# ghostop14/gr-clenabled

Measured on AMD Instinct MI355X. Metric: MSamples/sec (complex-float) through clFFT 4096 fwd + window + shift, higher is better.
Workload: dtype f32; 1 GPU; BASELINE configs[1]: forward clFFT 4096-pt complex, blackman window + fftshift, 16384 frames/step/GPU device-resident (1 GiB in+out); fft_size=4096, parallelism=replica-per-gpu x1

## Files before the change

gr-clenabled_amd/csrc/fft.hip:

```cpp
#include <cmath>
#include <cstdlib>
#include <vector>

#include "common.h"
#include "fft_core.hpp"
#include "fft_mr.h"

using namespace fftc;
#ifndef MI355_FFT_WPE
#define MI355_FFT_WPE 3
#endif

namespace {

typedef float f2v __attribute__((ext_vector_type(2)));

template <int N, bool REAL, class G>
__device__ __forceinline__ void load_group(c32 (&v)[16], const void *__restrict__ in, int grp, int tid, int nframes, int in_xor)
{
    using P = Plan<N>;
    constexpr int TH = G::TH, PTS = G::PTS, F = G::F, R0 = P::radix(0), B0 = N / R0;
    const int frames_left = nframes - grp * F;
    if constexpr (N <= 64) {
        (void)in_xor;
// ... 496 lines not shown
template <int N>
int launch_s(mi355_ctx *ctx, int sign, const void *in, void *out, const float *window, const void *tw, int nframes, int shift,
             int real_in, hipStream_t st)
{
    const int grid = N == 32768   ? mi355_balanced_grid(ctx, nframes, 1, 1)
                     : N == 16384 ? mi355_balanced_grid(ctx, nframes, 16, 16)
                                  : mi355_balanced_grid(ctx, nframes, 4, 4);
    if constexpr (N == 32768) {
        if (!getenv("MI355_FFT_32768_IN_REGISTERS")) {
#define LAUNCH_32K(SG, RL) hipLaunchKernelGGL((k_fft_32k<SG, RL>), dim3(grid), dim3(512), 0, st, in, (c32 *)out, window, (const c32 *)tw, nframes, shift)
            if (sign < 0) { if (real_in) LAUNCH_32K(-1, true); else LAUNCH_32K(-1, false); }
            else          { if (real_in) LAUNCH_32K(1, true);  else LAUNCH_32K(1, false); }
#undef LAUNCH_32K
            MI355_HIP(hipGetLastError());
            return MI355_OK;
        }
    }
    if constexpr (N == 32768) MI355_SWITCH_NOTE(ctx, "MI355_FFT_32768_IN_REGISTERS", "k_fft_s<32768> instead of k_fft_32k");
#define LAUNCH_S(SG, RL) hipLaunchKernelGGL((k_fft_s<N, SG, RL>), dim3(grid), dim3(256), 0, st, in, (c32 *)out, window, (const c32 *)tw, nframes, shift)
    if (sign < 0) { if (real_in) LAUNCH_S(-1, true); else LAUNCH_S(-1, false); }
    else          { if (real_in) LAUNCH_S(1, true);  else LAUNCH_S(1, false); }
#undef LAUNCH_S
    MI355_HIP(hipGetLastError());
    return MI355_OK;
}

template <int SIGN, bool REAL>
__global__ __launch_bounds__(256, 2) void k_fft_sub(const void *__restrict__ in, c32 *__restrict__ ws, const float *__restrict__ window,
                                                    const c32 *__restrict__ tw4096, int S, int nquad , int in_xor)
{
    constexpr int NS = 4096, BL = 256, Q = 4;
    using G = Geo<NS>;
    __shared__ c32 lds[NS];
    const int tid0 = threadIdx.x;
    const int per = S / Q, nframes = nquad / per;
    const int xcd = blockIdx.x & 7, per_xcd = gridDim.x >> 3;
    for (int q = blockIdx.x >> 3;; q += per_xcd) {
        const int frame = (q / per) * 8 + xcd, s = Q * (q % per);
        if (q / per >= (nframes + 7) / 8) break;
        if (frame >= nframes) continue;
        int tid = tid0;
        asm volatile("" : "+v"(tid));
        const size_t fb = (size_t)frame * NS * S;
        c32 v[Q][16];
#pragma unroll
        for (int r = 0; r < 16; r++) {
            const int n = tid + ((r ^ in_xor) * BL);
            const size_t e = (size_t)n * S + s;
            const f4v w = *((const f4v *)window + (size_t)(s >> 2) * NS + n);
            if constexpr (REAL) {
                const f4v x = *(const f4v *)((const float *)in + fb + e);
                v[0][r] = mk(x.x * w.x, 0.f);
                v[1][r] = mk(x.y * w.y, 0.f);
                v[2][r] = mk(x.z * w.z, 0.f);
                v[3][r] = mk(x.w * w.w, 0.f);
            } else {
                const f4v x0 = *(const f4v *)((const c32 *)in + fb + e);
                const f4v x1 = *((const f4v *)((const c32 *)in + fb + e) + 1);
                v[0][r] = mk(x0.x * w.x, x0.y * w.x);
                v[1][r] = mk(x0.z * w.y, x0.w * w.y);
                v[2][r] = mk(x1.x * w.z, x1.y * w.z);
                v[3][r] = mk(x1.z * w.w, x1.w * w.w);
            }
        }
        TwRegs<NS> tw;
        load_twiddles<NS, false, G>(tw, tid, tw4096);
#define MI355_SUBQ(K)                                                                                                   \
        {                                                                                                              \
            transform_regs<NS, SIGN, false, G>(v[K], tw, lds, tid);                                                    \
            f2v *__restrict__ o = (f2v *)ws + ((size_t)frame * S + s + K) * NS + tid;                                  \
            _Pragma("unroll") for (int t = 0; t < 16; t++) {                                                           \
                f2v z;                                                                                                 \
                z.x = v[K][t].x;                                                                                       \
                z.y = v[K][t].y;                                                                                       \
                o[orev<16>(t) * BL] = z;                            \
            }                                                                                                          \
            __syncthreads();                                                                                           \
        }
        MI355_SUBQ(0) MI355_SUBQ(1) MI355_SUBQ(2) MI355_SUBQ(3)
#undef MI355_SUBQ
    }
}

template <int S, int SIGN>
__global__ __launch_bounds__(256) void k_fft_combine(const c32 *__restrict__ ws, c32 *__restrict__ out, const c32 *__restrict__ twN,
                                                     long long total , int m_xor)
{
    constexpr int NS = 4096, N = NS * S;
    for (long long e = (long long)blockIdx.x * 256 + threadIdx.x; e < total; e += (long long)gridDim.x * 256) {
        const long long frame = e / NS;
        const int k = (int)(e - frame * NS);
        const c32 *src = ws + (size_t)frame * N + k;
        c32 a[S];
#pragma unroll
        for (int s = 0; s < S; s++) a[s] = src[(size_t)s * NS];
        c32 wsl[tw_slots<S>()];
#pragma unroll
        for (int i = 0; i < tw_slots<S>(); i++) wsl[i] = twN[(tw_power<S>(i) * k) & (N - 1)];
        apply_twiddles<S>(a, wsl);
        bfly<S, SIGN>(a);
        f2v *dst = (f2v *)out + (size_t)frame * N + k;
#pragma unroll
        for (int t = 0; t < S; t++) {
            f2v z;
            z.x = a[t].x;
            z.y = a[t].y;
            __builtin_nontemporal_store(z, dst + (size_t)((orev<S>(t) ^ m_xor) * NS));
        }
    }
}

template <int S, int SIGN>
__global__ __launch_bounds__(256) void k_fft_combine2(const c32 *__restrict__ src, c32 *__restrict__ dst, const c32 *__restrict__ twN,
                                                      long long total , int nsub, long long frame_elems, long long src_sub,
                                                      long long src_set, long long dst_set, int tw_mul, int nmask, int m_xor)
{
    const int set = blockIdx.y;
    for (long long e = (long long)blockIdx.x * 256 + threadIdx.x; e < total; e += (long long)gridDim.x * 256) {
        const long long frame = e / nsub;
        const int k = (int)(e - frame * nsub);
        const c32 *in = src + (size_t)frame * frame_elems + (size_t)set * src_set + k;
        c32 a[S];
#pragma unroll
        for (int s = 0; s < S; s++) a[s] = in[(size_t)s * src_sub];
        c32 wsl[tw_slots<S>()];
#pragma unroll
        for (int i = 0; i < tw_slots<S>(); i++) wsl[i] = twN[(int)(((long long)tw_power<S>(i) * k * tw_mul) & nmask)];
        apply_twiddles<S>(a, wsl);
        bfly<S, SIGN>(a);
        f2v *out = (f2v *)dst + (size_t)frame * frame_elems + (size_t)set * dst_set + k;
#pragma unroll
        for (int t = 0; t < S; t++) {
            f2v z;
            z.x = a[t].x;
            z.y = a[t].y;
            out[(size_t)((orev<S>(t) ^ m_xor)) * nsub] = z;
        }
    }
}

template <int NR> struct GeoTile {
    static constexpr int TH = NR, PTS = 16 * NR, F = 16, WPE = 1;
};

template <int NR, int SIGN, bool PASS_B, bool REAL, bool WR>
__global__ __launch_bounds__(NR, 4) void k_fft_tile(const void *__restrict__ in, c32 *__restrict__ out, const float *__restrict__ window,
                                                 const c32 *__restrict__ twN, const c32 *__restrict__ twR,
                                                 int ld , int nmask ,
                                                 long long nitems , int row_xor)
{
    using G = GeoTile<NR>;
    constexpr bool REV = !PASS_B;
    using PL = Plan<NR, REV>;
    constexpr int TH = NR, CS = NR + 1;
    extern __shared__ __attribute__((aligned(16))) c32 tile_lds[];
    const int tid0 = threadIdx.x;
    TwRegs<NR> tw;
    load_twiddles<NR, REV, G>(tw, tid0, twR);
    const int tiles = ld / 16;
    const size_t frame_elems = (size_t)NR * ld;
    constexpr bool WREG = !PASS_B && WR;
    float wreg[16];
    int c0_window = -1;
    for (long long item = blockIdx.x; item < nitems; item += gridDim.x) {
        int tid = tid0;
        asm volatile("" : "+v"(tid));
        const long long frame = item / tiles;
        const int c0 = (int)(item - frame * tiles) * 16;
        if constexpr (WREG) {
            if (c0 != c0_window) {
#pragma unroll
                for (int i = 0; i < 16; i++) {
                    const int e = tid + TH * i, col = e & 15, row = e >> 4;
                    wreg[i] = window[(size_t)(row ^ row_xor) * ld + c0 + col];
                }
                c0_window = c0;
            }
        }
#pragma unroll
        for (int i = 0; i < 16; i++) {
            const int e = tid + TH * i, col = e & 15, row = e >> 4;
            const size_t idx = (size_t)(PASS_B ? row : (row ^ row_xor)) * ld + c0 + col;
            c32 x;
            if constexpr (REAL) x = mk(((const float *)in)[(size_t)frame * frame_elems + idx], 0.f);
            else {
                const f2v t = __builtin_nontemporal_load((const f2v *)in + (size_t)frame * frame_elems + idx);
                x = mk(t.x, t.y);
            }
            if constexpr (!PASS_B) {
                const float w = WREG ? wreg[i] : window[idx];
                x = mk(x.x * w, x.y * w);
            }
            tile_lds[col * CS + row] = x;
        }
        __syncthreads();
        c32 v[16];
        constexpr int R0 = PL::radix(0), B0 = NR / R0;
#pragma unroll
        for (int q = 0; q < 16 / R0; q++) {
            const int g = tid + TH * q, fr = g / B0, j = g % B0;
#pragma unroll
            for (int r = 0; r < R0; r++) v[q * R0 + r] = tile_lds[fr * CS + j + r * B0];
        }
        __syncthreads();
        transform_regs<NR, SIGN, REV, G>(v, tw, tile_lds, tid);
        constexpr int NP = PL::NP, RL = PL::radix(NP - 1), BL = NR / RL;
        if constexpr (!PASS_B) {
            static_assert(RL == 16, "reversed plan: the last pass is radix 16");
            const int fr = tid / BL, j = tid % BL, n2 = c0 + fr;
            const c32 base = twN[(int)(((long long)n2 * j) & nmask)], g1 = twN[(int)(((long long)n2 * BL) & nmask)];
            const c32 g2 = cmul(g1, g1), g4 = cmul(g2, g2), g8 = cmul(g4, g4);
            c32 gp[16];
            gp[0] = base;
            gp[1] = cmul(base, g1);
            gp[2] = cmul(base, g2);
            gp[3] = cmul(gp[2], g1);
            gp[4] = cmul(base, g4);
            gp[5] = cmul(gp[4], g1);
            gp[6] = cmul(gp[4], g2);
            gp[7] = cmul(gp[6], g1);
#pragma unroll
            for (int m = 0; m < 8; m++) gp[8 + m] = cmul(gp[m], g8);
            f2v *__restrict__ o = (f2v *)out + (size_t)frame * frame_elems + (size_t)n2 * NR + j;
#pragma unroll
            for (int t = 0; t < 16; t++) {
                const c32 z = cmul(v[t], gp[orev<16>(t)]);
                f2v zz;
                zz.x = z.x;
                zz.y = z.y;
                o[orev<16>(t) * BL] = zz;
            }
            __syncthreads();
        } else {
            __syncthreads();
#pragma unroll
            for (int q = 0; q < 16 / RL; q++) {
                const int g = tid + TH * q, fr = g / BL, j = g % BL;
#pragma unroll
                for (int t = 0; t < RL; t++) tile_lds[fr * CS + j + orev<RL>(t) * BL] = v[q * RL + t];
            }
            __syncthreads();
#pragma unroll
            for (int i = 0; i < 16; i++) {
                const int e = tid + TH * i, col = e & 15, row = e >> 4;
                const c32 z = tile_lds[col * CS + row];
                f2v zz;
                zz.x = z.x;
                zz.y = z.y;
                __builtin_nontemporal_store(zz, (f2v *)out + (size_t)frame * frame_elems + (size_t)(row ^ row_xor) * ld + c0 + col);
            }
            __syncthreads();
        }
    }
}

template <int NR> struct GeoTileH {
    static constexpr int TH = NR / 2, PTS = 8 * NR, F = 8, WPE = 1;
};

template <int NR, int SIGN, bool PASS_B, bool REAL>
__global__ __launch_bounds__(NR / 2) void k_fft_tile_h(const void *__restrict__ in, c32 *__restrict__ out, const float *__restrict__ window,
                                                       const c32 *__restrict__ twN, const c32 *__restrict__ twR, int ld, int nmask,
                                                       long long nitems, int row_xor)
{
    using G = GeoTileH<NR>;
    constexpr bool REV = !PASS_B;
    using PL = Plan<NR, REV>;
    constexpr int TH = NR / 2, CS = NR + 1;
    extern __shared__ __attribute__((aligned(16))) c32 tile_lds[];
    const int tid0 = threadIdx.x;
    TwRegs<NR> tw;
    load_twiddles<NR, REV, G>(tw, tid0, twR);
    const int tiles = ld / 16;
    const size_t frame_elems = (size_t)NR * ld;
    auto fetch = [&](long long item, c32 (&pf)[32], int tid) {
        const long long frame = item / tiles;
        const int c0 = (int)(item - frame * tiles) * 16;
#pragma unroll
        for (int i = 0; i < 32; i++) {
            const int e = tid + TH * i, col = e & 15, row = e >> 4;
            const size_t idx = (size_t)(PASS_B ? row : (row ^ row_xor)) * ld + c0 + col;
            if constexpr (REAL) pf[i] = mk(((const float *)in)[(size_t)frame * frame_elems + idx], 0.f);
            else {
                const f2v t = __builtin_nontemporal_load((const f2v *)in + (size_t)frame * frame_elems + idx);
                pf[i] = mk(t.x, t.y);
            }
        }
    };
    c32 pf[32];
    if ((long long)blockIdx.x < nitems) fetch(blockIdx.x, pf, tid0);
    for (long long item = blockIdx.x; item < nitems; item += gridDim.x) {
        int tid = tid0;
        asm volatile("" : "+v"(tid));
        const long long frame = item / tiles;
        const int c0 = (int)(item - frame * tiles) * 16;
#pragma unroll
        for (int i = 0; i < 32; i++) {
            const int e = tid + TH * i, col = e & 15, row = e >> 4;
            c32 x = pf[i];
            if constexpr (!PASS_B) {
                const float w = window[(size_t)(row ^ row_xor) * ld + c0 + col];
                x = mk(x.x * w, x.y * w);
            }
            tile_lds[col * CS + row] = x;
        }
        __syncthreads();
        c32 va[16], vb[16];
        constexpr int R0 = PL::radix(0), B0 = NR / R0;
#pragma unroll
        for (int q = 0; q < 16 / R0; q++) {
            const int g = tid + TH * q, fr = g / B0, j = g % B0;
#pragma unroll
            for (int r = 0; r < R0; r++) {
                va[q * R0 + r] = tile_lds[fr * CS + j + r * B0];
                vb[q * R0 + r] = tile_lds[(fr + 8) * CS + j + r * B0];
            }
        }
        __syncthreads();
        if (item + gridDim.x < nitems) fetch(item + gridDim.x, pf, tid);
        transform_regs2<NR, SIGN, REV, G>(va, vb, tw, tile_lds, tile_lds + 8 * NR, tid);
        constexpr int NP = PL::NP, RL = PL::radix(NP - 1), BL = NR / RL;
        if constexpr (!PASS_B) {
            static_assert(RL == 16, "reversed plan: the last pass is radix 16");
            const int fr = tid / BL, j = tid % BL;
#pragma unroll
            for (int h = 0; h < 2; h++) {
                const int n2 = c0 + fr + 8 * h;
                const c32 base = twN[(int)(((long long)n2 * j) & nmask)], g1 = twN[(int)(((long long)n2 * BL) & nmask)];
                const c32 g2 = cmul(g1, g1), g4 = cmul(g2, g2), g8 = cmul(g4, g4);
                c32 gp[16];
                gp[0] = base;
                gp[1] = cmul(base, g1);
                gp[2] = cmul(base, g2);
                gp[3] = cmul(gp[2], g1);
                gp[4] = cmul(base, g4);
                gp[5] = cmul(gp[4], g1);
                gp[6] = cmul(gp[4], g2);
                gp[7] = cmul(gp[6], g1);
#pragma unroll
                for (int m = 0; m < 8; m++) gp[8 + m] = cmul(gp[m], g8);
                f2v *__restrict__ o = (f2v *)out + (size_t)frame * frame_elems + (size_t)n2 * NR + j;
#pragma unroll
                for (int t = 0; t < 16; t++) {
                    const c32 z = cmul(h ? vb[t] : va[t], gp[orev<16>(t)]);
                    f2v zz;
                    zz.x = z.x;
                    zz.y = z.y;
                    o[orev<16>(t) * BL] = zz;
                }
            }
            __syncthreads();
        } else {
            __syncthreads();
#pragma unroll
            for (int q = 0; q < 16 / RL; q++) {
                const int g = tid + TH * q, fr = g / BL, j = g % BL;
#pragma unroll
                for (int t = 0; t < RL; t++) {
                    tile_lds[fr * CS + j + orev<RL>(t) * BL] = va[q * RL + t];
                    tile_lds[(fr + 8) * CS + j + orev<RL>(t) * BL] = vb[q * RL + t];
                }
            }
            __syncthreads();
#pragma unroll
            for (int i = 0; i < 32; i++) {
                const int e = tid + TH * i, col = e & 15, row = e >> 4;
                const c32 z = tile_lds[col * CS + row];
                f2v zz;
                zz.x = z.x;
                zz.y = z.y;
                __builtin_nontemporal_store(zz, (f2v *)out + (size_t)frame * frame_elems + (size_t)(row ^ row_xor) * ld + c0 + col);
            }
            __syncthreads();
        }
    }
}

unsigned long long *stamps_buffer(int grid)
{
    static std::mutex mu;
    static unsigned long long *d = nullptr;
    static int cap = 0;
    std::lock_guard<std::mutex> g(mu);
    if (cap < grid) {
        if (d) (void)hipFree(d);
        d = nullptr;
        cap = 0;
        if (hipMalloc(&d, (size_t)grid * kTsSlots * 8) != hipSuccess) return nullptr;
        cap = grid;
    }
    return d;
}

int dump_stamps(const unsigned long long *d_ts, int n, int sign, int sched, int grid, int ngroups, hipStream_t st)
{
    MI355_HIP(hipStreamSynchronize(st));
    std::vector<unsigned long long> h((size_t)grid * kTsSlots);
    MI355_HIP(hipMemcpy(h.data(), d_ts, h.size() * 8, hipMemcpyDeviceToHost));
    unsigned long long t0 = ~0ull, t1 = 0;
    for (int b = 0; b < grid; b++) {
        t0 = std::min(t0, h[(size_t)b * kTsSlots]);
        t1 = std::max(t1, h[(size_t)b * kTsSlots + 1]);
    }
    fprintf(stderr, "[fft stamps] N %d sign %d sched %d: %d workgroups, %d groups, first start to last end %.2f us\n", n, sign, sched, grid,
            ngroups, (double)(t1 - t0) * 0.01);
    if (const char *path = getenv("MI355_FFT_TS_FILE")) {
        if (FILE *f = fopen(path, "a")) {
            fprintf(f, "# n %d sign %d sched %d grid %d ngroups %d\n", n, sign, sched, grid, ngroups);
            for (int b = 0; b < grid; b++) {
                const unsigned long long *r = &h[(size_t)b * kTsSlots];
                fprintf(f, "%d %llu %llu %llu %llu", b, r[3], r[0], r[1], r[2]);
                for (int i = 8; i < kTsSlots && r[i]; i++) fprintf(f, " %llu", r[i]);
                fprintf(f, "\n");
            }
            fclose(f);
        }
    }
    return MI355_OK;
}

template <int N, class G>
int launch_g(mi355_ctx *ctx, int sign, const void *in, void *out, const float *window, const void *tw, int nframes, int shift,
             int real_in, hipStream_t st, unsigned *claims)
{
    constexpr int F = G::F, TH = G::TH, WAVES = TH / 64;
    int ngroups = (nframes + F - 1) / F;
    int cus = ctx->num_cus > 0 ? ctx->num_cus : 256;
    int pf = getenv("MI355_FFT_PREFETCH") ? atoi(getenv("MI355_FFT_PREFETCH")) : -1;
    const bool persistent2 = N <= 4096 && WAVES == 4 && ngroups >= cus * 2 * 8;
    if (pf < 0) pf = persistent2 ? 1 : 0;
    int grid = (N <= 4096) ? mi355_balanced_grid(ctx, ngroups, 32 / WAVES, 64 / WAVES, 0.015) : mi355_balanced_grid(ctx, ngroups, 1, 1);
    if (pf == 1 && persistent2) grid = cus * 2;
    if (const char *e = getenv("MI355_FFT_WG_PER_CU")) {
        if (atoi(e) > 0) grid = ngroups < cus * atoi(e) ? ngroups : cus * atoi(e);
    }
    int sched = getenv("MI355_FFT_SCHED") ? atoi(getenv("MI355_FFT_SCHED")) : (N == 4096 ? 1 : 0);
    if (!(pf == 1 && persistent2 && claims && grid >= 8 * kClaimWords &&
          ngroups / kClaimWords >= kClaimStatic * ((grid + 8 * kClaimWords - 1) / (8 * kClaimWords)) * 8))
        sched = 0;
    if (sched != 1) claims = nullptr;
    unsigned long long *ts = nullptr;
    if (pf == 1 && getenv("MI355_FFT_TS")) {
        ts = stamps_buffer(grid);
        if (ts) MI355_HIP(hipMemsetAsync(ts, 0, (size_t)grid * kTsSlots * 8, st));
    }
#define LAUNCH_FFT_K(...) hipLaunchKernelGGL((k_fft<__VA_ARGS__>), dim3(grid), dim3(TH), 0, st, in, (c32 *)out, window, (const c32 *)tw, \
                                                nframes, ngroups, shift, claims, ts)
#define LAUNCH_FFT(SG, RL)                                                                      \
    do {                                                                                             \
        if (pf == 2) LAUNCH_FFT_K(N, SG, RL, 2, G);                                                  \
        else if (pf == 1 && sched == 1 && ts) LAUNCH_FFT_K(N, SG, RL, 1, G, true, true);             \
        else if (pf == 1 && sched == 1) LAUNCH_FFT_K(N, SG, RL, 1, G, true);                         \
        else if (pf == 1 && ts) LAUNCH_FFT_K(N, SG, RL, 1, G, false, true);                          \
        else if (pf == 1) LAUNCH_FFT_K(N, SG, RL, 1, G);                                             \
        else LAUNCH_FFT_K(N, SG, RL, 0, G);                                                          \
    } while (0)
    if (sign < 0) { if (real_in) LAUNCH_FFT(-1, true); else LAUNCH_FFT(-1, false); }
    else          { if (real_in) LAUNCH_FFT(1, true);  else LAUNCH_FFT(1, false); }
#undef LAUNCH_FFT
#undef LAUNCH_FFT_K
    MI355_HIP(hipGetLastError());
    if (ts) return dump_stamps(ts, N, sign, sched, grid, ngroups, st);
    return MI355_OK;
}

template <int N>
int launch_n(mi355_ctx *ctx, int sign, const void *in, void *out, const float *window, const void *tw, int nframes, int shift,
             int real_in, hipStream_t st, unsigned *claims)
{
    if constexpr (N >= 16 && N <= 1024) {
        static const bool wave = getenv("MI355_FFT_WAVE_GEO") ? atoi(getenv("MI355_FFT_WAVE_GEO")) != 0 : false;
        if (wave) MI355_SWITCH_NOTE(ctx, "MI355_FFT_WAVE_GEO", "k_fft in one-wave workgroups");
        if (wave) return launch_g<N, GeoW<N>>(ctx, sign, in, out, window, tw, nframes, shift, real_in, st, claims);
    }
    if constexpr (N == 32768) return launch_s<N>(ctx, sign, in, out, window, tw, nframes, shift, real_in, st);
    else if constexpr (N == 8192 || N == 16384) {
        static const bool whole = getenv("MI355_FFT_WHOLE_FRAME") ? atoi(getenv("MI355_FFT_WHOLE_FRAME")) != 0 : false;
        if (!whole) return launch_s<N>(ctx, sign, in, out, window, tw, nframes, shift, real_in, st);
        MI355_SWITCH_NOTE(ctx, "MI355_FFT_WHOLE_FRAME", "k_fft with the whole frame in LDS instead of k_fft_s");
    }
    if constexpr (N != 32768) return launch_g<N, Geo<N>>(ctx, sign, in, out, window, tw, nframes, shift, real_in, st, claims);
}

int launch_fft(mi355_ctx *ctx, int n, int sign, const void *in, void *out, const float *window, const void *tw, int nframes,
               int shift, int real_in, hipStream_t st, unsigned *claims = nullptr)
{
    switch (n) {
#define CASE_N(NN) case NN: return launch_n<NN>(ctx, sign, in, out, window, tw, nframes, shift, real_in, st, claims)
        CASE_N(2); CASE_N(4); CASE_N(8); CASE_N(16); CASE_N(32); CASE_N(64); CASE_N(128); CASE_N(256); CASE_N(512);
        CASE_N(1024); CASE_N(2048); CASE_N(4096); CASE_N(8192); CASE_N(16384); CASE_N(32768);
#undef CASE_N
    }
    mi355_set_error("fft size %d unsupported (power of two, 2..32768)", n);
    return MI355_ERR_UNSUPPORTED;
}

}

struct mi355_fft {
    mi355_ctx *ctx;
    int n, sign, dtype, nstreams, shift;
    float *d_window;
    void *d_tw;
    HostPipe pipe;
    MrPlan mr;
    MrTilePlan mrt;
    int m = 0;
    void *d_pre = nullptr, *d_post = nullptr, *d_bspec = nullptr;
    void *d_twm_f = nullptr, *d_twm_i = nullptr;
    float *d_ones = nullptr;
    mi355_fft *sub_f = nullptr, *sub_i = nullptr;
    void *d_wa = nullptr, *d_wb = nullptr;
    size_t cap_frames = 0;
    bool two_kernel = false;
    int tile_n1 = 0, tile_n2 = 0;
    std::mutex ws_lock;
    hipEvent_t ws_done = nullptr;
    bool ws_used = false;
    unsigned *d_claims = nullptr;
    hipStream_t claim_st[kClaimSets] = {};
// ... 83 lines not shown
                    if constexpr (REAL) x = mk(((const float *)in)[(fbase + fr) * N + i], 0.f);
                    else x = ((const c32 *)in)[(fbase + fr) * N + i];
                    x = cmul(x, pre[m]);
                }
                v[q * R0 + r] = x;
            }
        }
        transform_regs<M, -1, false, G>(v, twf, lds, tid);
        c32 w[16];
#pragma unroll
        for (int q = 0; q < 16 / RL; q++)
#pragma unroll
            for (int r = 0; r < RL; r++) w[q * RL + r] = cmul(v[q * RL + irev<RL>(r)], Breg[q * RL + irev<RL>(r)]);
        if constexpr (NP > 1) __syncthreads();
        if constexpr (SHARE) transform_regs<M, 1, true, G, 0, true>(w, twf, lds, tid);
        else transform_regs<M, 1, true, G>(w, twi, lds, tid);
        constexpr int RO = PI::radix(NP - 1), BO = M / RO;
#pragma unroll
        for (int q = 0; q < 16 / RO; q++) {
            const int g = tid + TH * q, fr = g / BO, j = g % BO;
#pragma unroll
            for (int t = 0; t < RO; t++) {
                const int k = j + orev<RO>(t) * BO;
                if (k < N && fr < frames_left) {
                    const int p = lo ? (k >= lo ? k - lo : k + (N - lo)) : k;
                    out[(fbase + fr) * N + p] = cmul(w[q * RO + t], post[k]);
                }
            }
        }
        if constexpr (NP > 1) __syncthreads();
    }
}

template <int M>
int launch_chirpz_m(mi355_fft *h, const void *in, void *out, int nframes, hipStream_t st)
{
    constexpr int F = Geo<M>::F, TH = Geo<M>::TH;
    const int ngroups = (nframes + F - 1) / F;
    const int grid = mi355_balanced_grid(h->ctx, ngroups, 2, 3);
    const int lo = (h->sign < 0 && h->shift) ? (h->n + 1) / 2 : 0;
    const int *src = (const int *)((const char *)h->d_post + (size_t)h->n * 8);
    constexpr int lds_bytes = Geo<M>::PTS * 8;
    if (h->dtype == MI355_DTYPE_FLOAT) {
        if (lds_bytes > 64 * 1024) MI355_HIP(hipFuncSetAttribute((const void *)k_chirpz<M, true>, hipFuncAttributeMaxDynamicSharedMemorySize, lds_bytes));
        hipLaunchKernelGGL((k_chirpz<M, true>), dim3(grid), dim3(TH), lds_bytes, st, in, (c32 *)out, (const c32 *)h->d_pre, src, (const c32 *)h->d_post,
                           (const c32 *)h->d_bspec, (const c32 *)h->d_twm_f, (const c32 *)h->d_twm_i, h->n, nframes, ngroups, lo);
    } else {
        if (lds_bytes > 64 * 1024) MI355_HIP(hipFuncSetAttribute((const void *)k_chirpz<M, false>, hipFuncAttributeMaxDynamicSharedMemorySize, lds_bytes));
        hipLaunchKernelGGL((k_chirpz<M, false>), dim3(grid), dim3(TH), lds_bytes, st, in, (c32 *)out, (const c32 *)h->d_pre, src, (const c32 *)h->d_post,
                           (const c32 *)h->d_bspec, (const c32 *)h->d_twm_f, (const c32 *)h->d_twm_i, h->n, nframes, ngroups, lo);
    }
    MI355_HIP(hipGetLastError());
    return MI355_OK;
}

int ws_acquire(mi355_fft *h, hipStream_t st, bool realloc)
{
    if (!h->ws_done) MI355_HIP(hipEventCreateWithFlags(&h->ws_done, hipEventDisableTiming));
    if (h->ws_used) {
        if (realloc) MI355_HIP(hipEventSynchronize(h->ws_done));
        else MI355_HIP(hipStreamWaitEvent(st, h->ws_done, 0));
    }
    return MI355_OK;
}
int ws_release(mi355_fft *h, hipStream_t st)
{
    MI355_HIP(hipEventRecord(h->ws_done, st));
    h->ws_used = true;
    return MI355_OK;
}

int launch_handle(mi355_fft *h, const void *in, void *out, int nvec, hipStream_t st);

int launch_bluestein(mi355_fft *h, const void *in, void *out, int nframes, hipStream_t st)
{
    const int N = h->n, M = h->m;
    static const bool fused = getenv("MI355_CHIRPZ_FUSED") ? atoi(getenv("MI355_CHIRPZ_FUSED")) != 0 : true;
    if (fused) {
        switch (M) {
        case 256: return launch_chirpz_m<256>(h, in, out, nframes, st);
        case 512: return launch_chirpz_m<512>(h, in, out, nframes, st);
        case 1024: return launch_chirpz_m<1024>(h, in, out, nframes, st);
        case 2048: return launch_chirpz_m<2048>(h, in, out, nframes, st);
        case 4096: return launch_chirpz_m<4096>(h, in, out, nframes, st);
        case 8192: return launch_chirpz_m<8192>(h, in, out, nframes, st);
        case 16384: return launch_chirpz_m<16384>(h, in, out, nframes, st);
        }
    }
    if (!fused && M >= 256 && M <= 16384) MI355_SWITCH_NOTE(h->ctx, "MI355_CHIRPZ_FUSED", "the five-launch chirp-z path instead of k_chirpz");
    size_t chunk = (128u << 20) / ((size_t)M * 8);
    if (chunk < 1) chunk = 1;
    if (chunk > (size_t)nframes) chunk = (size_t)nframes;
    std::lock_guard<std::mutex> ws_guard(h->ws_lock);
    {
        const int rc = ws_acquire(h, st, chunk > h->cap_frames);
        if (rc) return rc;
    }
    if (chunk > h->cap_frames) {
        MI355_HIP(hipStreamSynchronize(st));
        if (h->d_wa) (void)hipFree(h->d_wa);
        if (h->d_wb) (void)hipFree(h->d_wb);
        h->d_wa = h->d_wb = nullptr; h->cap_frames = 0;
        MI355_HIP(hipMalloc(&h->d_wa, chunk * (size_t)M * 8));
        MI355_HIP(hipMalloc(&h->d_wb, chunk * (size_t)M * 8));
        h->cap_frames = chunk;
    }
    const int cus = h->ctx->num_cus > 0 ? h->ctx->num_cus : 256;
    auto grid_for = [&](long long total) { long long b = (total + 255) / 256; return (unsigned)(b < (long long)cus * 16 ? b : (long long)cus * 16); };
    const size_t isz = h->dtype == MI355_DTYPE_FLOAT ? 4 : 8;
    const int len = (N + 1) / 2;
    for (size_t f0 = 0; f0 < (size_t)nframes; f0 += chunk) {
        const int nf = (int)((size_t)nframes - f0 < chunk ? (size_t)nframes - f0 : chunk);
        const long long tm = (long long)nf * M, tn = (long long)nf * N;
        hipLaunchKernelGGL(k_blu_pre, dim3(grid_for(tm)), dim3(256), 0, st, (const char *)in + f0 * N * isz, (c32 *)h->d_wa,
                           (const c32 *)h->d_pre, (const int *)((const char *)h->d_post + (size_t)N * 8), N, M, tm,
                           h->dtype == MI355_DTYPE_FLOAT ? 1 : 0);
        int rc = h->sub_f ? launch_handle(h->sub_f, h->d_wa, h->d_wb, nf, st) : launch_fft(h->ctx, M, -1, h->d_wa, h->d_wb, h->d_ones, h->d_twm_f, nf, 0, 0, st);
        if (rc) return rc;
        hipLaunchKernelGGL(k_blu_mul, dim3(grid_for(tm)), dim3(256), 0, st, (c32 *)h->d_wb, (const c32 *)h->d_bspec, M, tm);
        rc = h->sub_i ? launch_handle(h->sub_i, h->d_wb, h->d_wa, nf, st) : launch_fft(h->ctx, M, 1, h->d_wb, h->d_wa, h->d_ones, h->d_twm_i, nf, 0, 0, st);
        if (rc) return rc;
        hipLaunchKernelGGL(k_blu_post, dim3(grid_for(tn)), dim3(256), 0, st, (const c32 *)h->d_wa, (c32 *)out + f0 * N,
                           (const c32 *)h->d_post, N, M, tn, (h->sign < 0 && h->shift) ? len : 0);
        MI355_HIP(hipGetLastError());
    }
    return ws_release(h, st);
}

template <int NR, bool PASS_B>
int launch_tile(mi355_fft *h, const void *in, c32 *out, const c32 *twR, int ld, int nframes, int row_xor, bool real_in, hipStream_t st)
{
    constexpr int lds_bytes = 16 * (NR + 1) * 8;
    const int cus = h->ctx->num_cus > 0 ? h->ctx->num_cus : 256;
    const long long items = (long long)nframes * (ld / 16);
    const int per_cu = (160 * 1024) / lds_bytes;
    long long grid = (long long)cus * (per_cu < 1 ? 1 : per_cu);
    if (grid > items) grid = items;
    if (grid > ld / 16) grid -= grid % (ld / 16);
    const int nmask = h->n - 1;
    constexpr bool WRD = !PASS_B && NR == 256;
    const bool wr = !PASS_B && NR < 1024 && (getenv("MI355_FFT_TILE_WREG") ? atoi(getenv("MI355_FFT_TILE_WREG")) != 0 : WRD);
#define TILE1(SG, RL, WR)                                                                                                       \
    do {                                                                                                                        \
        MI355_HIP(hipFuncSetAttribute((const void *)k_fft_tile<NR, SG, PASS_B, RL, WR>, hipFuncAttributeMaxDynamicSharedMemorySize, lds_bytes)); \
        hipLaunchKernelGGL((k_fft_tile<NR, SG, PASS_B, RL, WR>), dim3((unsigned)grid), dim3(NR), lds_bytes, st, in, out, h->d_window, (const c32 *)h->d_tw, \
                           twR, ld, nmask, items, row_xor);                                                                     \
    } while (0)
#define TILE(SG, RL)                                                                                                            \
    do {                                                                                                                        \
        if constexpr (!PASS_B && NR < 1024) { if (wr) TILE1(SG, RL, true); else TILE1(SG, RL, false); }                         \
        else TILE1(SG, RL, false);                                                                                              \
    } while (0)
    if constexpr (NR == 1024) {
        static const bool half = getenv("MI355_FFT_TILE_HALF") ? atoi(getenv("MI355_FFT_TILE_HALF")) != 0 : true;
        if (!half) MI355_SWITCH_NOTE(h->ctx, "MI355_FFT_TILE_HALF", "k_fft_tile with one thread per sixteen values instead of k_fft_tile_h");
        if (half) {
#define TILEH(SG, RL)                                                                                                           \
    do {                                                                                                                        \
        MI355_HIP(hipFuncSetAttribute((const void *)k_fft_tile_h<NR, SG, PASS_B, RL>, hipFuncAttributeMaxDynamicSharedMemorySize, lds_bytes)); \
        hipLaunchKernelGGL((k_fft_tile_h<NR, SG, PASS_B, RL>), dim3((unsigned)grid), dim3(NR / 2), lds_bytes, st, in, out, h->d_window, (const c32 *)h->d_tw, \
                           twR, ld, nmask, items, row_xor);                                                                     \
    } while (0)
            if constexpr (PASS_B) {
                if (h->sign < 0) TILEH(-1, false); else TILEH(1, false);
            } else {
                if (h->sign < 0) { if (real_in) TILEH(-1, true); else TILEH(-1, false); }
                else             { if (real_in) TILEH(1, true);  else TILEH(1, false); }
            }
#undef TILEH
            MI355_HIP(hipGetLastError());
            return MI355_OK;
        }
    }
    if constexpr (PASS_B) {
        if (h->sign < 0) TILE(-1, false); else TILE(1, false);
    } else {
        if (h->sign < 0) { if (real_in) TILE(-1, true); else TILE(-1, false); }
        else             { if (real_in) TILE(1, true);  else TILE(1, false); }
    }
#undef TILE
#undef TILE1
    (void)wr;
    MI355_HIP(hipGetLastError());
    return MI355_OK;
}

template <bool PASS_B>
int launch_tile_nr(mi355_fft *h, int nr, const void *in, c32 *out, const c32 *twR, int ld, int nframes, int row_xor, bool real_in, hipStream_t st)
{
    switch (nr) {
    case 256: return launch_tile<256, PASS_B>(h, in, out, twR, ld, nframes, row_xor, real_in, st);
    case 512: return launch_tile<512, PASS_B>(h, in, out, twR, ld, nframes, row_xor, real_in, st);
    default: return launch_tile<1024, PASS_B>(h, in, out, twR, ld, nframes, row_xor, real_in, st);
    }
}

int launch_big(mi355_fft *h, const void *in, void *out, int nframes, hipStream_t st)
{
    const int N = h->n, S = N / 4096;
    static const size_t ws_mb = getenv("MI355_FFT_WS_MB") ? (size_t)atoi(getenv("MI355_FFT_WS_MB")) : 256;
    if (ws_mb != 256) MI355_SWITCH_NOTE(h->ctx, "MI355_FFT_WS_MB", "another workspace bound for the multi-pass sizes");
    size_t chunk = (ws_mb << 20) / ((size_t)N * 8);
    if (chunk < 1) chunk = 1;
    if (chunk > (size_t)nframes) chunk = (size_t)nframes;
    std::lock_guard<std::mutex> ws_guard(h->ws_lock);
    {
        const int rc = ws_acquire(h, st, chunk > h->cap_frames);
        if (rc) return rc;
    }
    const bool three_pass = S > 16 && !h->tile_n1;
    const bool four_pass = S > 256;
    if (chunk > h->cap_frames) {
        MI355_HIP(hipStreamSynchronize(st));
        if (h->d_wa) (void)hipFree(h->d_wa);
        if (h->d_wb) (void)hipFree(h->d_wb);
        h->d_wa = h->d_wb = nullptr; h->cap_frames = 0;
        MI355_HIP(hipMalloc(&h->d_wa, chunk * (size_t)N * 8));
        if (three_pass) MI355_HIP(hipMalloc(&h->d_wb, chunk * (size_t)N * 8));
        h->cap_frames = chunk;
    }
    const int cus = h->ctx->num_cus > 0 ? h->ctx->num_cus : 256;
    const size_t isz = h->dtype == MI355_DTYPE_FLOAT ? 4 : 8;
    const int in_xor = (h->sign > 0 && h->shift) ? 8 : 0, m_xor = (h->sign < 0 && h->shift) ? S / 2 : 0;
    const c32 *tw4096 = (const c32 *)h->d_tw + N;
    for (size_t f0 = 0; f0 < (size_t)nframes; f0 += chunk) {
        const int nf = (int)((size_t)nframes - f0 < chunk ? (size_t)nframes - f0 : chunk);
        const int nsub = nf * S / 4;
        const int grid = (mi355_balanced_grid(h->ctx, nsub, 8, 8) + 7) & ~7;
        const void *src = (const char *)in + f0 * N * isz;
        if (h->tile_n1) {
            const int n1 = h->tile_n1, n2 = h->tile_n2;
            const c32 *tw1 = (const c32 *)h->d_tw + N + 4096, *tw2 = tw1 + n1;
            int rc = launch_tile_nr<false>(h, n1, src, (c32 *)h->d_wa, tw1, n2, nf, (h->sign > 0 && h->shift) ? n1 / 2 : 0, h->dtype == MI355_DTYPE_FLOAT, st);
            if (rc) return rc;
            rc = launch_tile_nr<true>(h, n2, h->d_wa, (c32 *)out + f0 * N, tw2, n1, nf, (h->sign < 0 && h->shift) ? n2 / 2 : 0, false, st);
            if (rc) return rc;
            continue;
        }
#define SUB(SG, RL) hipLaunchKernelGGL((k_fft_sub<SG, RL>), dim3(grid), dim3(256), 0, st, src, (c32 *)h->d_wa, h->d_window, tw4096, S, nsub, in_xor)
        if (h->sign < 0) { if (h->dtype == MI355_DTYPE_FLOAT) SUB(-1, true); else SUB(-1, false); }
        else             { if (h->dtype == MI355_DTYPE_FLOAT) SUB(1, true);  else SUB(1, false); }
#undef SUB
        c32 *dst = (c32 *)out + f0 * N;
#define COMB2(SS, SG, GY, ...) hipLaunchKernelGGL((k_fft_combine2<SS, SG>), dim3((unsigned)blocks, GY), dim3(256), 0, st, __VA_ARGS__)
        if (four_pass) {
            const int S3 = S / 256, T2 = 16 * S3;
            {
                const long long total = (long long)nf * 4096;
                long long blocks = (total + 255) / 256;
                if (blocks > (long long)cus * 16 / T2 + 1) blocks = (long long)cus * 16 / T2 + 1;
                if (h->sign < 0) COMB2(16, -1, T2, (const c32 *)h->d_wa, (c32 *)h->d_wb, (const c32 *)h->d_tw, total, 4096, (long long)N, (long long)T2 * 4096, 4096LL, 65536LL, T2, N - 1, 0);
                else             COMB2(16, 1, T2, (const c32 *)h->d_wa, (c32 *)h->d_wb, (const c32 *)h->d_tw, total, 4096, (long long)N, (long long)T2 * 4096, 4096LL, 65536LL, T2, N - 1, 0);
            }
            {
                const long long total = (long long)nf * 65536;
                long long blocks = (total + 255) / 256;
                if (blocks > (long long)cus * 16 / S3 + 1) blocks = (long long)cus * 16 / S3 + 1;
                if (h->sign < 0) COMB2(16, -1, S3, (const c32 *)h->d_wb, (c32 *)h->d_wa, (const c32 *)h->d_tw, total, 65536, (long long)N, (long long)S3 * 65536, 65536LL, 1048576LL, S3, N - 1, 0);
                else             COMB2(16, 1, S3, (const c32 *)h->d_wb, (c32 *)h->d_wa, (const c32 *)h->d_tw, total, 65536, (long long)N, (long long)S3 * 65536, 65536LL, 1048576LL, S3, N - 1, 0);
            }
            {
                const long long total = (long long)nf * 1048576;
                long long blocks = (total + 255) / 256;
                if (blocks > (long long)cus * 16) blocks = (long long)cus * 16;
                const int mx = (h->sign < 0 && h->shift) ? S3 / 2 : 0;
#define COMB2G(SS) do { if (h->sign < 0) COMB2(SS, -1, 1, (const c32 *)h->d_wa, dst, (const c32 *)h->d_tw, total, 1048576, (long long)N, 1048576LL, 0LL, 0LL, 1, N - 1, mx); \
                        else             COMB2(SS, 1, 1, (const c32 *)h->d_wa, dst, (const c32 *)h->d_tw, total, 1048576, (long long)N, 1048576LL, 0LL, 0LL, 1, N - 1, mx); } while (0)
                if (S3 == 2) COMB2G(2); else if (S3 == 4) COMB2G(4); else if (S3 == 8) COMB2G(8); else COMB2G(16);
#undef COMB2G
            }
            MI355_HIP(hipGetLastError());
            continue;
        }
        if (three_pass) {
            const int S2 = S / 16;
            {
                const long long total = (long long)nf * 4096;
                long long blocks = (total + 255) / 256;
                if (blocks > (long long)cus * 16 / S2 + 1) blocks = (long long)cus * 16 / S2 + 1;
                if (h->sign < 0) COMB2(16, -1, S2, (const c32 *)h->d_wa, (c32 *)h->d_wb, (const c32 *)h->d_tw, total, 4096, (long long)N, (long long)S2 * 4096, 4096LL, 65536LL, S2, N - 1, 0);
                else             COMB2(16, 1, S2, (const c32 *)h->d_wa, (c32 *)h->d_wb, (const c32 *)h->d_tw, total, 4096, (long long)N, (long long)S2 * 4096, 4096LL, 65536LL, S2, N - 1, 0);
            }
            {
                const long long total = (long long)nf * 65536;
                long long blocks = (total + 255) / 256;
                if (blocks > (long long)cus * 16) blocks = (long long)cus * 16;
                const int mx = (h->sign < 0 && h->shift) ? S2 / 2 : 0;
#define COMB2F(SS) do { if (h->sign < 0) COMB2(SS, -1, 1, (const c32 *)h->d_wb, dst, (const c32 *)h->d_tw, total, 65536, (long long)N, 65536LL, 0LL, 0LL, 1, N - 1, mx); \
                        else             COMB2(SS, 1, 1, (const c32 *)h->d_wb, dst, (const c32 *)h->d_tw, total, 65536, (long long)N, 65536LL, 0LL, 0LL, 1, N - 1, mx); } while (0)
                if (S2 == 2) COMB2F(2); else if (S2 == 4) COMB2F(4); else if (S2 == 8) COMB2F(8); else COMB2F(16);
#undef COMB2F
            }
            MI355_HIP(hipGetLastError());
            continue;
        }
#undef COMB2
        const long long total = (long long)nf * 4096;
        long long blocks = (total + 255) / 256;
        if (blocks > (long long)cus * 16) blocks = (long long)cus * 16;
#define COMB(SS, SG) hipLaunchKernelGGL((k_fft_combine<SS, SG>), dim3((unsigned)blocks), dim3(256), 0, st, (const c32 *)h->d_wa, dst, (const c32 *)h->d_tw, total, m_xor)
        if (S == 8) { if (h->sign < 0) COMB(8, -1); else COMB(8, 1); }
        else        { if (h->sign < 0) COMB(16, -1); else COMB(16, 1); }
#undef COMB
        MI355_HIP(hipGetLastError());
    }
    return ws_release(h, st);
}

// ... 437 lines not shown
```

gr-clenabled_amd/csrc/fft_core.hpp:

```cpp
#pragma once
#include <hip/hip_runtime.h>

namespace fftc {

struct c32 { float x, y; };

__device__ __forceinline__ c32 mk(float x, float y) { c32 r; r.x = x; r.y = y; return r; }
__device__ __forceinline__ c32 operator+(c32 a, c32 b) { return mk(a.x + b.x, a.y + b.y); }
__device__ __forceinline__ c32 operator-(c32 a, c32 b) { return mk(a.x - b.x, a.y - b.y); }
__device__ __forceinline__ c32 cmul(c32 a, c32 b) { return mk(a.x * b.x - a.y * b.y, a.x * b.y + a.y * b.x); }
__device__ __forceinline__ c32 cconj(c32 a) { return mk(a.x, -a.y); }
__device__ __forceinline__ c32 scale(c32 a, float s) { return mk(a.x * s, a.y * s); }
template <int SIGN> __device__ __forceinline__ c32 rot90(c32 a) { return SIGN < 0 ? mk(a.y, -a.x) : mk(-a.y, a.x); }
template <int SIGN> __device__ __forceinline__ c32 rot45(c32 a)
{
    constexpr float h = 0.70710678118654752440f;
    return SIGN < 0 ? mk((a.x + a.y) * h, (a.y - a.x) * h) : mk((a.x - a.y) * h, (a.y + a.x) * h);
}
template <int SIGN> __device__ __forceinline__ c32 rot135(c32 a)
{
    constexpr float h = 0.70710678118654752440f;
    return SIGN < 0 ? mk((a.y - a.x) * h, -(a.x + a.y) * h) : mk(-(a.x + a.y) * h, (a.x - a.y) * h);
}
template <int SIGN, int M> __device__ __forceinline__ c32 rot16(c32 a)
// ... 100 lines not shown
    static constexpr int PTS = TH * 16;
    static constexpr int F = PTS / N;
    static constexpr int WPE = 2;
};

__host__ __device__ constexpr int swz(int s) { return s ^ ((s >> 4) & 15); }

template <int N> __host__ __device__ constexpr int swzn(int s)
{
    if (N == 256) return s ^ ((s >> 4) & 31);
    if (N == 64) return s ^ ((s >> 4) & 15) ^ ((((s >> 6) ^ (s >> 8)) & 1) << 4);
    return swz(s);
}

template <int STEP, int N = 0> __device__ __forceinline__ int lds_at(int raw, int raw_swz, int c)
{
    (void)raw;
    if constexpr (STEP % 256 == 0 && N != 256 && N != 64) return raw_swz + c;
    else return raw_swz ^ swzn<N>(c);
}

template <int STEP, int N = 0> __device__ __forceinline__ c32 &lds_slot(c32 *lds, int raw_swz8, int c)
{
    if constexpr (STEP % 256 == 0 && N != 256 && N != 64) return *(c32 *)((char *)lds + raw_swz8 + c * 8);
    else return *(c32 *)((char *)lds + (raw_swz8 ^ (swzn<N>(c) * 8)));
}

template <int R> __host__ __device__ constexpr int irev(int r)
{
    if (R == 16) return (r >> 2) + 4 * (r & 3);
    if (R == 8) return (r & 1) * 4 + (r >> 1);
    return r;
}

template <int R> __host__ __device__ constexpr int tw_slots() { return R == 16 ? 6 : R == 8 ? 4 : R == 4 ? 3 : 1; }
template <int R> __host__ __device__ constexpr int tw_power(int i) { return i < 3 ? i + 1 : (i - 2) * 4; }
constexpr int kTwPerPass = 12;
template <int N> struct TwRegs { c32 w[Plan<N>::NP > 1 ? Plan<N>::NP - 1 : 1][kTwPerPass]; };

template <int N, bool REV, class G = Geo<N>, int P = 1>
__device__ __forceinline__ void load_twiddles(TwRegs<N> &tw, int tid, const c32 *__restrict__ twtab)
{
    using PL = Plan<N, REV>;
    if constexpr (P < PL::NP) {
        constexpr int TH = G::TH, R = PL::radix(P), NS = PL::ns(P), B = N / R, S = tw_slots<R>();
#pragma unroll
        for (int q = 0; q < 16 / R; q++) {
            const int j = (tid + TH * q) % B, k = j % NS;
#pragma unroll
            for (int i = 0; i < S; i++) tw.w[P - 1][q * S + i] = twtab[(tw_power<R>(i) * k * (N / (NS * R))) & (N - 1)];
        }
        load_twiddles<N, REV, G, P + 1>(tw, tid, twtab);
    }
}

template <int R, bool CJ = false> __device__ __forceinline__ void apply_twiddles(c32 *v, const c32 *w_in)
{
    c32 w[tw_slots<R>()];
#pragma unroll
    for (int i = 0; i < tw_slots<R>(); i++) {
        w[i] = w_in[i];
        if (CJ) w[i].y = -w[i].y;
        asm volatile("" : "+v"(w[i].x), "+v"(w[i].y));
    }
#pragma unroll
    for (int r = 1; r < R; r++) {
        const int lo = r & 3, hi = r >> 2;
        c32 t;
        if (hi == 0) t = w[lo - 1];
        else if (lo == 0) t = w[2 + hi];
        else t = cmul(w[2 + hi], w[lo - 1]);
        v[r] = cmul(v[r], t);
    }
}

template <int N, int SIGN, bool REV, class G = Geo<N>, int P = 0, bool CJ = false>
__device__ __forceinline__ void transform_regs(c32 (&v)[16], const TwRegs<N> &tw, c32 *lds, int tid)
{
    using PL = Plan<N, REV>;
    if constexpr (P < PL::NP) {
        constexpr int TH = G::TH, NP = PL::NP, R = PL::radix(P), NS = PL::ns(P), B = N / R;
        if constexpr (P > 0) {
            __syncthreads();
#pragma unroll
            for (int q = 0; q < 16 / R; q++) {
                const int g = tid + TH * q, raw = (g / B) * N + (g % B), rs8 = swzn<N>(raw) * 8;
#pragma unroll
                for (int r = 0; r < R; r++) v[q * R + r] = lds_slot<B, N>(lds, rs8, r * B);
            }
#pragma unroll
            for (int q = 0; q < 16 / R; q++) apply_twiddles<R, CJ>(&v[q * R], &tw.w[P - 1][q * tw_slots<R>()]);
            if constexpr (P < NP - 1) __syncthreads();
        }
#pragma unroll
        for (int q = 0; q < 16 / R; q++) bfly<R, SIGN>(&v[q * R]);
        if constexpr (P < NP - 1) {
#pragma unroll
            for (int q = 0; q < 16 / R; q++) {
                const int g = tid + TH * q, fr = g / B, j = g % B;
                const int raw = fr * N + (j / NS) * NS * R + (j % NS), rs8 = swzn<N>(raw) * 8;
#pragma unroll
                for (int s = 0; s < R; s++) lds_slot<NS, N>(lds, rs8, orev<R>(s) * NS) = v[q * R + s];
            }
        }
        transform_regs<N, SIGN, REV, G, P + 1, CJ>(v, tw, lds, tid);
    }
}

template <int N, int SIGN, bool REV, class G = Geo<N>, int P = 0, bool CJ = false>
__device__ __forceinline__ void transform_regs2(c32 (&va)[16], c32 (&vb)[16], const TwRegs<N> &tw, c32 *lds_a, c32 *lds_b, int tid)
{
    using PL = Plan<N, REV>;
    if constexpr (P < PL::NP) {
        constexpr int TH = G::TH, NP = PL::NP, R = PL::radix(P), NS = PL::ns(P), B = N / R;
        if constexpr (P > 0) {
            __syncthreads();
#pragma unroll
            for (int q = 0; q < 16 / R; q++) {
                const int g = tid + TH * q, raw = (g / B) * N + (g % B), rs = swzn<N>(raw);
#pragma unroll
                for (int r = 0; r < R; r++) {
                    va[q * R + r] = lds_a[lds_at<B, N>(raw, rs, r * B)];
                    vb[q * R + r] = lds_b[lds_at<B, N>(raw, rs, r * B)];
                }
            }
#pragma unroll
            for (int q = 0; q < 16 / R; q++) {
                apply_twiddles<R, CJ>(&va[q * R], &tw.w[P - 1][q * tw_slots<R>()]);
                apply_twiddles<R, CJ>(&vb[q * R], &tw.w[P - 1][q * tw_slots<R>()]);
            }
            if constexpr (P < NP - 1) __syncthreads();
        }
#pragma unroll
        for (int q = 0; q < 16 / R; q++) {
            bfly<R, SIGN>(&va[q * R]);
            bfly<R, SIGN>(&vb[q * R]);
        }
        if constexpr (P < NP - 1) {
#pragma unroll
            for (int q = 0; q < 16 / R; q++) {
                const int g = tid + TH * q, fr = g / B, j = g % B;
                const int raw = fr * N + (j / NS) * NS * R + (j % NS), rs = swzn<N>(raw);
#pragma unroll
                for (int s = 0; s < R; s++) {
                    lds_a[lds_at<NS, N>(raw, rs, orev<R>(s) * NS)] = va[q * R + s];
                    lds_b[lds_at<NS, N>(raw, rs, orev<R>(s) * NS)] = vb[q * R + s];
                }
            }
        }
        transform_regs2<N, SIGN, REV, G, P + 1, CJ>(va, vb, tw, lds_a, lds_b, tid);
    }
}

}
```

Before: 389,200 MSamples/s.

## Fold column-major tile transposes into FFT passes, drop extra LDS round trips

The tiled 1024-point FFT kernels used to write loaded columns to a padded LDS tile, sync, and read them back before the transform. Pass B did the same again before storing. A new transform_cm now keeps the column-major data in registers and reads and writes a swizzled LDS layout inside the first and last passes, which removes two LDS transposes and their barriers per tile. The half-thread variant shares the same path with prefetch-friendly address math and is no longer the default, so k_fft_tile now runs by default. The changes add complex swizzle indexing and the risk of bank conflicts or extra register pressure, and they disable FP contraction on the window multiply.

```diff
diff --git a/gr-clenabled_amd/csrc/fft.hip b/gr-clenabled_amd/csrc/fft.hip
--- a/gr-clenabled_amd/csrc/fft.hip
+++ b/gr-clenabled_amd/csrc/fft.hip
@@ -672,11 +672,12 @@
     using G = GeoTile<NR>;
     constexpr bool REV = !PASS_B;
     using PL = Plan<NR, REV>;
-    constexpr int TH = NR, CS = NR + 1;
+    constexpr int TH = NR;
     extern __shared__ __attribute__((aligned(16))) c32 tile_lds[];
     const int tid0 = threadIdx.x;
-    TwRegs<NR> tw;
-    load_twiddles<NR, REV, G>(tw, tid0, twR);
+    TwRegs<NR> tw[1];
+    load_twiddles<NR, REV, G>(tw[0], tid0, twR);
+    if constexpr (PASS_B) load_twiddles_cm_last<NR, REV>(tw[0], tid0, twR);
     const int tiles = ld / 16;
     const size_t frame_elems = (size_t)NR * ld;
     constexpr bool WREG = !PASS_B && WR;
@@ -697,6 +698,9 @@
                 c0_window = c0;
             }
         }
+        c32 vv[1][16];
+        c32(&v)[16] = vv[0];
+        constexpr int R0 = PL::radix(0);
 #pragma unroll
         for (int i = 0; i < 16; i++) {
             const int e = tid + TH * i, col = e & 15, row = e >> 4;
@@ -708,22 +712,13 @@
                 x = mk(t.x, t.y);
             }
             if constexpr (!PASS_B) {
+#pragma clang fp contract(off)
                 const float w = WREG ? wreg[i] : window[idx];
                 x = mk(x.x * w, x.y * w);
             }
-            tile_lds[col * CS + row] = x;
-        }
-        __syncthreads();
-        c32 v[16];
-        constexpr int R0 = PL::radix(0), B0 = NR / R0;
-#pragma unroll
-        for (int q = 0; q < 16 / R0; q++) {
-            const int g = tid + TH * q, fr = g / B0, j = g % B0;
-#pragma unroll
-            for (int r = 0; r < R0; r++) v[q * R0 + r] = tile_lds[fr * CS + j + r * B0];
-        }
-        __syncthreads();
-        transform_regs<NR, SIGN, REV, G>(v, tw, tile_lds, tid);
+            v[(i % (16 / R0)) * R0 + i / (16 / R0)] = x;
+        }
+        transform_cm<NR, SIGN, REV, PASS_B, G>(vv, tw, tile_lds, tid);
         constexpr int NP = PL::NP, RL = PL::radix(NP - 1), BL = NR / RL;
         if constexpr (!PASS_B) {
             static_assert(RL == 16, "reversed plan: the last pass is radix 16");
@@ -752,18 +747,10 @@
             }
             __syncthreads();
         } else {
-            __syncthreads();
-#pragma unroll
-            for (int q = 0; q < 16 / RL; q++) {
-                const int g = tid + TH * q, fr = g / BL, j = g % BL;
-#pragma unroll
-                for (int t = 0; t < RL; t++) tile_lds[fr * CS + j + orev<RL>(t) * BL] = v[q * RL + t];
-            }
-            __syncthreads();
 #pragma unroll
             for (int i = 0; i < 16; i++) {
                 const int e = tid + TH * i, col = e & 15, row = e >> 4;
-                const c32 z = tile_lds[col * CS + row];
+                const c32 z = v[(i % (16 / RL)) * RL + irev<RL>(i / (16 / RL))];
                 f2v zz;
                 zz.x = z.x;
                 zz.y = z.y;
@@ -774,35 +761,31 @@
     }
 }
 
-template <int NR> struct GeoTileH {
-    static constexpr int TH = NR / 2, PTS = 8 * NR, F = 8, WPE = 1;
-};
-
 template <int NR, int SIGN, bool PASS_B, bool REAL>
 __global__ __launch_bounds__(NR / 2) void k_fft_tile_h(const void *__restrict__ in, c32 *__restrict__ out, const float *__restrict__ window,
                                                        const c32 *__restrict__ twN, const c32 *__restrict__ twR, int ld, int nmask,
                                                        long long nitems, int row_xor)
 {
-    using G = GeoTileH<NR>;
+    using G = GeoTile<NR>;
     constexpr bool REV = !PASS_B;
     using PL = Plan<NR, REV>;
-    constexpr int TH = NR / 2, CS = NR + 1;
+    constexpr int TH = NR / 2;
     extern __shared__ __attribute__((aligned(16))) c32 tile_lds[];
     const int tid0 = threadIdx.x;
-    TwRegs<NR> tw;
-    load_twiddles<NR, REV, G>(tw, tid0, twR);
+    TwRegs<NR> tw[2];
+    load_twiddles<NR, REV, G>(tw[0], tid0, twR);
     const int tiles = ld / 16;
     const size_t frame_elems = (size_t)NR * ld;
     auto fetch = [&](long long item, c32 (&pf)[32], int tid) {
         const long long frame = item / tiles;
         const int c0 = (int)(item - frame * tiles) * 16;
+        const unsigned lane = (unsigned)(tid >> 4) * (unsigned)ld + (unsigned)(tid & 15);
 #pragma unroll
         for (int i = 0; i < 32; i++) {
-            const int e = tid + TH * i, col = e & 15, row = e >> 4;
-            const size_t idx = (size_t)(PASS_B ? row : (row ^ row_xor)) * ld + c0 + col;
-            if constexpr (REAL) pf[i] = mk(((const float *)in)[(size_t)frame * frame_elems + idx], 0.f);
+            const size_t u = (size_t)frame * frame_elems + (size_t)(PASS_B ? (TH / 16) * i : ((TH / 16) * i) ^ row_xor) * ld + c0;
+            if constexpr (REAL) pf[i] = mk(((const float *)in + u)[lane], 0.f);
             else {
-                const f2v t = __builtin_nontemporal_load((const f2v *)in + (size_t)frame * frame_elems + idx);
+                const f2v t = __builtin_nontemporal_load((const f2v *)in + u + lane);
                 pf[i] = mk(t.x, t.y);
             }
         }
@@ -814,31 +797,28 @@
         asm volatile("" : "+v"(tid));
         const long long frame = item / tiles;
         const int c0 = (int)(item - frame * tiles) * 16;
+        c32 v[2][16];
+        constexpr int R0 = PL::radix(0);
 #pragma unroll
         for (int i = 0; i < 32; i++) {
             const int e = tid + TH * i, col = e & 15, row = e >> 4;
             c32 x = pf[i];
             if constexpr (!PASS_B) {
+#pragma clang fp contract(off)
                 const float w = window[(size_t)(row ^ row_xor) * ld + c0 + col];
                 x = mk(x.x * w, x.y * w);
             }
-            tile_lds[col * CS + row] = x;
-        }
-        __syncthreads();
-        c32 va[16], vb[16];
-        constexpr int R0 = PL::radix(0), B0 = NR / R0;
-#pragma unroll
-        for (int q = 0; q < 16 / R0; q++) {
-            const int g = tid + TH * q, fr = g / B0, j = g % B0;
-#pragma unroll
-            for (int r = 0; r < R0; r++) {
-                va[q * R0 + r] = tile_lds[fr * CS + j + r * B0];
-                vb[q * R0 + r] = tile_lds[(fr + 8) * CS + j + r * B0];
-            }
-        }
-        __syncthreads();
+            v[i & 1][((i >> 1) % (16 / R0)) * R0 + (i >> 1) / (16 / R0)] = x;
+            if constexpr (!PASS_B) {
+                if (i == 15) __builtin_amdgcn_sched_barrier(0);
+            }
+        }
         if (item + gridDim.x < nitems) fetch(item + gridDim.x, pf, tid);
-        transform_regs2<NR, SIGN, REV, G>(va, vb, tw, tile_lds, tile_lds + 8 * NR, tid);
+        if constexpr (PASS_B) {
+            load_twiddles_cm_last<NR, REV>(tw[0], tid, twR);
+            load_twiddles_cm_last<NR, REV>(tw[1], tid + TH, twR);
+        } else load_twiddles<NR, REV, G, PL::NP - 1>(tw[0], tid, twR);
+        transform_cm<NR, SIGN, REV, PASS_B, G, 2>(v, tw, tile_lds, tid);
         constexpr int NP = PL::NP, RL = PL::radix(NP - 1), BL = NR / RL;
         if constexpr (!PASS_B) {
             static_assert(RL == 16, "reversed plan: the last pass is radix 16");
@@ -862,7 +842,7 @@
                 f2v *__restrict__ o = (f2v *)out + (size_t)frame * frame_elems + (size_t)n2 * NR + j;
 #pragma unroll
                 for (int t = 0; t < 16; t++) {
-                    const c32 z = cmul(h ? vb[t] : va[t], gp[orev<16>(t)]);
+                    const c32 z = cmul(v[h][t], gp[orev<16>(t)]);
                     f2v zz;
                     zz.x = z.x;
                     zz.y = z.y;
@@ -871,21 +851,10 @@
             }
             __syncthreads();
         } else {
-            __syncthreads();
-#pragma unroll
-            for (int q = 0; q < 16 / RL; q++) {
-                const int g = tid + TH * q, fr = g / BL, j = g % BL;
-#pragma unroll
-                for (int t = 0; t < RL; t++) {
-                    tile_lds[fr * CS + j + orev<RL>(t) * BL] = va[q * RL + t];
-                    tile_lds[(fr + 8) * CS + j + orev<RL>(t) * BL] = vb[q * RL + t];
-                }
-            }
-            __syncthreads();
 #pragma unroll
             for (int i = 0; i < 32; i++) {
                 const int e = tid + TH * i, col = e & 15, row = e >> 4;
-                const c32 z = tile_lds[col * CS + row];
+                const c32 z = v[i & 1][((i >> 1) % (16 / RL)) * RL + irev<RL>((i >> 1) / (16 / RL))];
                 f2v zz;
                 zz.x = z.x;
                 zz.y = z.y;
@@ -1275,8 +1244,9 @@
         else TILE1(SG, RL, false);                                                                                              \
     } while (0)
     if constexpr (NR == 1024) {
-        static const bool half = getenv("MI355_FFT_TILE_HALF") ? atoi(getenv("MI355_FFT_TILE_HALF")) != 0 : true;
-        if (!half) MI355_SWITCH_NOTE(h->ctx, "MI355_FFT_TILE_HALF", "k_fft_tile with one thread per sixteen values instead of k_fft_tile_h");
+        static const char *half_env = getenv("MI355_FFT_TILE_HALF");
+        static const bool half = half_env ? atoi(half_env) != 0 : false;
+        if (half_env) MI355_SWITCH_NOTE(h->ctx, "MI355_FFT_TILE_HALF", half ? "k_fft_tile_h, half the threads" : "k_fft_tile with one thread per sixteen values, not k_fft_tile_h");
         if (half) {
 #define TILEH(SG, RL)                                                                                                           \
     do {                                                                                                                        \
diff --git a/gr-clenabled_amd/csrc/fft_core.hpp b/gr-clenabled_amd/csrc/fft_core.hpp
--- a/gr-clenabled_amd/csrc/fft_core.hpp
+++ b/gr-clenabled_amd/csrc/fft_core.hpp
@@ -276,4 +276,90 @@
     }
 }
 
-}
+__host__ __device__ constexpr int cmx(int c) { return c ^ ((c & 1) << 4); }
+
+template <int STEP> __device__ __forceinline__ c32 &cm_slot(c32 *lds, int base8, int c)
+{
+    if constexpr (STEP % 32 == 0) return *(c32 *)((char *)lds + base8 + c * 8);
+    else return *(c32 *)((char *)lds + (base8 ^ (c * 8)));
+}
+
+template <int N, bool REV> __device__ __forceinline__ void load_twiddles_cm_last(TwRegs<N> &tw, int tid, const c32 *__restrict__ twtab)
+{
+    using PL = Plan<N, REV>;
+    constexpr int P = PL::NP - 1, R = PL::radix(P), S = tw_slots<R>();
+    static_assert(PL::ns(P) * R == N, "last stage");
+#pragma unroll
+    for (int q = 0; q < 16 / R; q++) {
+        const int j = (tid >> 4) + q * (N / 16);
+#pragma unroll
+        for (int i = 0; i < S; i++) tw.w[P - 1][q * S + i] = twtab[(tw_power<R>(i) * j) & (N - 1)];
+    }
+}
+
+template <int N, int SIGN, bool REV, bool CM_OUT, class G, int NV = 1, int P = 0>
+__device__ __forceinline__ void transform_cm(c32 (&v)[NV][16], const TwRegs<N> (&tw)[NV], c32 *lds, int tid)
+{
+    using PL = Plan<N, REV>;
+    static_assert(G::TH == N && G::F == 16 && PL::NP >= 2, "sixteen columns, one (virtual) thread per sixteen values");
+    if constexpr (P < PL::NP) {
+        constexpr int TH = G::TH, NP = PL::NP, R = PL::radix(P), NS = PL::ns(P), B = N / R;
+        static_assert((N / NV) % B == 0 && (N / NV) % 16 == 0, "virtual threads share the row twiddles and the column");
+        constexpr bool RD_CM = CM_OUT && P == NP - 1, RD_X = P == 1 || RD_CM;
+        constexpr bool WR_CM = P == 0, WR_X = WR_CM || (CM_OUT && P == NP - 2);
+        if constexpr (P > 0) {
+            __syncthreads();
+#pragma unroll
+            for (int q = 0; q < 16 / R; q++) {
+#pragma unroll
+                for (int k = 0; k < NV; k++) {
+                    const int tv = tid + k * (N / NV), g = tv + TH * q;
+                    const int fr = RD_CM ? (tv & 15) : g / B, j = RD_CM ? (tv >> 4) + q * (N / 16) : g % B;
+                    if constexpr (RD_X) {
+                        const int b8 = (fr * N + (j ^ cmx(fr))) * 8;
+#pragma unroll
+                        for (int r = 0; r < R; r++) v[k][q * R + r] = cm_slot<B>(lds, b8, r * B);
+                    } else {
+                        const int rs8 = swzn<N>(fr * N + j) * 8;
+#pragma unroll
+                        for (int r = 0; r < R; r++) v[k][q * R + r] = lds_slot<B, N>(lds, rs8, r * B);
+                    }
+                }
+            }
+#pragma unroll
+            for (int q = 0; q < 16 / R; q++) {
+#pragma unroll
+                for (int k = 0; k < NV; k++) apply_twiddles<R>(&v[k][q * R], &tw[RD_CM ? k : 0].w[P - 1][q * tw_slots<R>()]);
+            }
+            if constexpr (P < NP - 1) __syncthreads();
+        }
+#pragma unroll
+        for (int q = 0; q < 16 / R; q++) {
+#pragma unroll
+            for (int k = 0; k < NV; k++) bfly<R, SIGN>(&v[k][q * R]);
+        }
+        if constexpr (P < NP - 1) {
+#pragma unroll
+            for (int q = 0; q < 16 / R; q++) {
+#pragma unroll
+                for (int k = 0; k < NV; k++) {
+                    const int tv = tid + k * (N / NV), g = tv + TH * q;
+                    const int fr = WR_CM ? (tv & 15) : g / B, j = WR_CM ? (tv >> 4) + q * (N / 16) : g % B;
+                    const int raw = fr * N + (j / NS) * NS * R + (j % NS);
+                    if constexpr (WR_X) {
+                        const int b8 = (raw ^ cmx(fr)) * 8;
+#pragma unroll
+                        for (int s = 0; s < R; s++) cm_slot<NS>(lds, b8, orev<R>(s) * NS) = v[k][q * R + s];
+                    } else {
+                        const int rs8 = swzn<N>(raw) * 8;
+#pragma unroll
+                        for (int s = 0; s < R; s++) lds_slot<NS, N>(lds, rs8, orev<R>(s) * NS) = v[k][q * R + s];
+                    }
+                }
+            }
+        }
+        transform_cm<N, SIGN, REV, CM_OUT, G, NV, P + 1>(v, tw, lds, tid);
+    }
+}
+
+}
```

Result: no change. 389,600 MSamples/s (median of 2 runs) (+0.1%).
